# radhofan/Fairify

Measured on AMD Instinct MI355X. Metric: % partitions verified + partitions/sec on AC suite at 1/2/4/8 MI355X, higher is better.
Workload: dtype fp32

## Files before the change

fairify_amd/csrc/bindings.cpp:

```cpp
#include <hip/hip_runtime.h>
#include <pybind11/pybind11.h>
#include <pybind11/stl.h>

#include <cmath>
#include <cstring>
#include <cstdint>
#include <stdexcept>
#include <vector>

#include "runtime_host.h"

namespace py = pybind11;

extern "C" int fa_bounds_launch(const NetDesc& net, BoundArgs args, hipStream_t stream);
extern "C" int fa_crown_phase_launch(const NetDesc& net, CrownPhaseArgs a, hipStream_t stream);
extern "C" size_t fa_crown_phase_bytes(const NetDesc& net);
extern "C" int fa_point_try_launch(const NetDesc& net, BoundArgs a, hipStream_t stream);
extern "C" int fa_forward_launch(const NetDesc& net, FwdArgs a, hipStream_t stream);
extern "C" int fa_sim_launch(const NetDesc& net, SimArgs a, hipStream_t stream);
extern "C" int fa_sim_shaped(const NetDesc& net);
extern "C" int fa_ascent_launch(const NetDesc& net, AscentArgs a, hipStream_t stream);
extern "C" int fa_certify_launch(CertArgs a, hipStream_t stream);
extern "C" int fa_falsify_launch(const NetDesc& net, FalsifyArgs a, hipStream_t stream);
extern "C" int fa_prune_masks_launch(const NetDesc& net, int P, const int* counts, const float* ub, int ub_stride,
// ... 317 lines not shown
    a.npa = (int)pa.size();
    for (size_t i = 0; i < pa.size(); ++i) a.pa_idx[i] = pa[i];
    a.values = P<const int64_t>(values);
    a.Pp = Pp;
    a.pairs = P<const int64_t>(pairs);
    a.nfree = (int)free_dims.size();
    for (size_t i = 0; i < free_dims.size(); ++i) a.free_idx[i] = free_dims[i];
    a.found = P<uint8_t>(found);
    a.wit_x = P<float>(wit_x);
    a.wit_xp = P<float>(wit_xp);
    const int rc = fa_ascent_launch(net.d, a, (hipStream_t)stream);
    if (rc == -1) return false;
    ckl(rc, "ascent");
    return true;
  });

  m.def("falsify", [](const Net& net, uintptr_t flat, uintptr_t lo, uintptr_t hi, uintptr_t pids, int Pn,
                      int n_samples, int n_local, uint32_t seed, int V, const std::vector<int>& pa, uintptr_t values,
                      int Pp, uintptr_t pairs, int walk_k, int walk_steps, int K, int iters,
                      const std::vector<int>& free_dims, uintptr_t found, uintptr_t wit_x, uintptr_t wit_xp,
                      uintptr_t how, uintptr_t stream, const std::vector<int>& ra, int tau, uint32_t dseed) {
    if (pa.size() > FA_MAX_PA || free_dims.size() > 64 || ra.size() > FA_MAX_RA)
      throw std::invalid_argument("too many PA/RA/free dims");
    FalsifyArgs a{};
    a.flat = P<const float>(flat);
    a.lo = P<const float>(lo);
    a.hi = P<const float>(hi);
    a.pids = P<const int64_t>(pids);
    a.P = Pn; a.n_samples = n_samples; a.n_local = n_local; a.seed = seed;
    a.V = V;
    a.npa = (int)pa.size();
    for (size_t i = 0; i < pa.size(); ++i) a.pa_idx[i] = pa[i];
    a.values = P<const int64_t>(values);
    a.Pp = Pp;
    a.pairs = P<const int64_t>(pairs);
    a.walk_k = walk_k; a.walk_steps = walk_steps; a.K = K; a.iters = iters;
    a.nfree = (int)free_dims.size();
    for (size_t i = 0; i < free_dims.size(); ++i) a.free_idx[i] = free_dims[i];
    a.found = P<uint8_t>(found);
    a.wit_x = P<float>(wit_x);
    a.wit_xp = P<float>(wit_xp);
    a.how = P<int8_t>(how);
    a.nra = tau > 0 ? (int)ra.size() : 0;
    for (int i = 0; i < a.nra; ++i) a.ra_idx[i] = ra[i];
    a.tau = tau;
    a.dseed = dseed;
    const int rc = fa_falsify_launch(net.d, a, (hipStream_t)stream);
    if (rc == 0) return false;
    if (rc < 0) ckl(-rc, "falsify");
    return true;
  });

  m.def("prune_masks", [](const Net& net, int Pn, uintptr_t counts, uintptr_t ub, int ub_stride, uintptr_t sym_dead,
                          uintptr_t code, uintptr_t cnt, uintptr_t stream) {
    ckl(fa_prune_masks_launch(net.d, Pn, P<const int>(counts), P<const float>(ub), ub_stride,
                                P<const uint8_t>(sym_dead), P<uint8_t>(code), P<int>(cnt), (hipStream_t)stream),
          "prune_masks");
  });

  m.def("heuristic", [](const Net& net, int Pu, uintptr_t rows, uintptr_t lb, uintptr_t ub, int stride, uintptr_t code,
                        double q50, double qlo, double qhi, uintptr_t hnew, uintptr_t hmerged, uintptr_t hcnt,
                        uintptr_t stream) {
    ckl(fa_heuristic_launch(net.d, Pu, P<const int64_t>(rows), P<const float>(lb), P<const float>(ub), stride,
                              P<const uint8_t>(code), q50, qlo, qhi, P<uint8_t>(hnew), P<uint8_t>(hmerged),
                              P<int>(hcnt), (hipStream_t)stream),
          "heuristic");
  });

  m.def("agree", [](const Net& net, uintptr_t flat, int Pm, uintptr_t rows, uintptr_t lo, uintptr_t hi, uintptr_t pids,
                    uintptr_t dead, int S, uint32_t seed, uintptr_t agree, uintptr_t stream) {
    const int rc = fa_agree_launch(net.d, P<const float>(flat), Pm, P<const int64_t>(rows), P<const float>(lo),
                                   P<const float>(hi), P<const int64_t>(pids), P<const uint8_t>(dead), S, seed,
                                   P<int>(agree), (hipStream_t)stream);
    if (rc == 0) return false;
    if (rc < 0) ckl(-rc, "agree");
    return true;
  });

  m.def("certify", [](int Nn, int n0, int V, int Pp, int norient, std::vector<uintptr_t> fx, std::vector<uintptr_t> fxp,
                      uintptr_t xlo, uintptr_t xhi, uintptr_t xplo, uintptr_t xphi, uintptr_t pairs, uintptr_t values,
                      const std::vector<int>& pa, const std::vector<int>& ra, double tau, uintptr_t shared,
                      double unit, double gmarg, uintptr_t gmin, uintptr_t tstar, uintptr_t open, uintptr_t score,
                      uintptr_t split_dim, uintptr_t cand_x, uintptr_t cand_xp, uintptr_t cand_v, uintptr_t cand_o,
                      uintptr_t scores, uintptr_t leaf, uintptr_t stream) {
    if (pa.size() > FA_CMAX_PA || ra.size() > FA_MAX_RA) throw std::invalid_argument("too many PA/RA dims");
    if (fx.size() != 8 || fxp.size() != 8) throw std::invalid_argument("need 8 form pointers (6 forms + lb/ub)");
    CertArgs a{};
    a.Nn = Nn; a.n0 = n0; a.V = V; a.Pp = Pp; a.norient = norient;
    a.Lc = P<const float>(fx[0]); a.L0 = P<const float>(fx[1]); a.Le = P<const float>(fx[2]);
    a.Uc = P<const float>(fx[3]); a.U0 = P<const float>(fx[4]); a.Ue = P<const float>(fx[5]);
    a.olb = P<const float>(fx[6]); a.oub = P<const float>(fx[7]);
    a.Lcp = P<const float>(fxp[0]); a.L0p = P<const float>(fxp[1]); a.Lep = P<const float>(fxp[2]);
    a.Ucp = P<const float>(fxp[3]); a.U0p = P<const float>(fxp[4]); a.Uep = P<const float>(fxp[5]);
    a.olbp = P<const float>(fxp[6]); a.oubp = P<const float>(fxp[7]);
    a.xlo = P<const float>(xlo); a.xhi = P<const float>(xhi);
    a.xplo = P<const float>(xplo); a.xphi = P<const float>(xphi);
    a.pairs = P<const int64_t>(pairs);
    a.values = P<const int64_t>(values);
    a.npa = (int)pa.size();
    for (size_t i = 0; i < pa.size(); ++i) a.pa_idx[i] = pa[i];
    a.nra = (int)ra.size();
    for (size_t i = 0; i < ra.size(); ++i) a.ra_idx[i] = ra[i];
    a.tau = (float)tau;
    a.shared = P<const uint8_t>(shared);
    a.unit = (float)unit;
    a.gmarg = std::nextafter((float)gmarg, INFINITY);
    a.gmin = P<float>(gmin); a.tstar = P<float>(tstar);
    a.open = P<uint8_t>(open); a.score = P<float>(score); a.split_dim = P<int64_t>(split_dim);
    a.cand_x = P<float>(cand_x); a.cand_xp = P<float>(cand_xp);
    a.cand_v = P<int64_t>(cand_v); a.cand_o = P<int64_t>(cand_o);
    a.scores = P<float>(scores); a.leaf = P<uint8_t>(leaf);
    ckl(fa_certify_launch(a, (hipStream_t)stream), "certify");
  });

  m.def("decode", [](std::vector<int> radix, std::vector<long long> div, std::vector<int> chunk_off,
                     std::vector<float> base_lo, std::vector<float> base_hi, uintptr_t ids, int Pn,
                     uintptr_t chunk_lo, uintptr_t chunk_hi, uintptr_t lo, uintptr_t hi, uintptr_t stream) {
    const size_t n0 = radix.size();
    if (n0 == 0 || n0 > FA_DECODE_MAX_DIMS || div.size() != n0 || chunk_off.size() != n0 || base_lo.size() != n0 ||
        base_hi.size() != n0)
      throw std::invalid_argument("decode: descriptor sizes");
    DecodeDesc d{};
    d.n0 = (int)n0;
    for (size_t k = 0; k < n0; ++k) {
      if (radix[k] < 0 || (radix[k] > 0 && div[k] <= 0)) throw std::invalid_argument("decode: radix/div");
      d.radix[k] = radix[k];
      d.div[k] = div[k];
      d.chunk_off[k] = chunk_off[k];
      d.base_lo[k] = base_lo[k];
      d.base_hi[k] = base_hi[k];
    }
    ckl(fa_decode_launch(d, P<const int64_t>(ids), Pn, P<const float>(chunk_lo), P<const float>(chunk_hi),
                           P<float>(lo), P<float>(hi), (hipStream_t)stream),
          "decode");
  });
  m.def("pack_masks", [](uintptr_t src, int Pn, int N, int stride, int sel, uintptr_t out, int NB, uintptr_t hash,
                         uintptr_t stream) {
    ckl(fa_pack_masks_launch(P<const uint8_t>(src), Pn, N, stride, sel, P<uint8_t>(out), NB,
                               P<unsigned long long>(hash), (hipStream_t)stream),
          "pack_masks");
  });
  m.def("knn", [](uintptr_t X, int n, int d, int k, uintptr_t idx, uintptr_t dist, uintptr_t stream) {
    ckl(fa_knn_launch(P<const float>(X), n, d, k, P<int>(idx), P<float>(dist), (hipStream_t)stream), "knn");
  });
  m.def("actdiff", [](const Net& net, uintptr_t flat, uintptr_t x, uintptr_t xp, int npairs, uintptr_t sum_out,
                      uintptr_t stream) {
    ckl(fa_actdiff_launch(net.d, P<const float>(flat), P<const float>(x), P<const float>(xp), npairs,
                            P<float>(sum_out), (hipStream_t)stream),
          "actdiff");
  });
  m.def("trace_marker", [](int tag, uintptr_t sink, uintptr_t stream) {
    ckl(fa_trace_marker_launch(tag, P<int>(sink), (hipStream_t)stream), "trace_marker");
  });
  auto beta_args = [](const Net& net, uintptr_t flat, uintptr_t wt, int R, const std::vector<int>& pa, uintptr_t lo,
                      uintptr_t hi, uintptr_t va, uintptr_t vb, uintptr_t LBA, uintptr_t UBA, uintptr_t LBB,
                      uintptr_t UBB, uintptr_t phA, uintptr_t phB, uintptr_t par, uintptr_t t, uintptr_t scratch,
                      int iters, float lr_a, float lr_b, float lr_t, float decay, int lookahead, int beta_pos,
                      int stall, uintptr_t bound, uintptr_t split, uintptr_t xstar, uintptr_t binit,
                      unsigned long long ramask, uintptr_t plo, uintptr_t phi, uintptr_t xpstar, uintptr_t gtie,
                      float tau, uintptr_t osg) {
    if (pa.size() > FA_MAX_PA) throw std::invalid_argument("beta_level: too many PA dims");
    for (size_t q = 0; q < pa.size(); ++q)
      if (pa[q] < 0 || pa[q] >= net.d.dims[0] || (q && pa[q] <= pa[q - 1]))
        throw std::invalid_argument("beta_level: PA dims must be increasing input indices");
    BetaArgs a;
    std::memset(&a, 0, sizeof(a));
    a.flat = P<const float>(flat);
    a.wt = P<const float>(wt);
    a.R = R;
    a.npa = (int)pa.size();
    for (size_t q = 0; q < pa.size(); ++q) a.pa_idx[q] = pa[q];
    a.lo = P<const float>(lo);
    a.hi = P<const float>(hi);
    a.va = P<const float>(va);
    a.vb = P<const float>(vb);
    a.LBA = P<const float>(LBA);
    a.UBA = P<const float>(UBA);
    a.LBB = P<const float>(LBB);
    a.UBB = P<const float>(UBB);
    a.phA = P<const int8_t>(phA);
    a.phB = P<const int8_t>(phB);
    a.par = P<float>(par);
    a.t = P<float>(t);
    a.scratch = P<float>(scratch);
    a.iters = iters;
    a.lr_a = lr_a;
    a.lr_b = lr_b;
    a.lr_t = lr_t;
    a.decay = decay;
    a.lookahead = lookahead;
    a.beta_pos = beta_pos;
    a.stall = stall & 1;
    a.pgap = (stall >> 1) & 3;
    a.feas = (stall >> 3) & 1;
// ... 113 lines not shown
```

fairify_amd/csrc/certify.hip:

```cpp
#include "args.h"

struct Form {
  const float* c;
  float c0;
  float fmag;
};

__device__ __forceinline__ bool fa_is_pa(const CertArgs& a, int d) {
  for (int k = 0; k < a.npa; ++k)
    if (a.pa_idx[k] == d) return true;
  return false;
}

__device__ __forceinline__ Form fa_fold(const CertArgs& a, const float* C, float c0, int v) {
  Form f;
  f.c = C;
  float contrib = 0.f, cmag = 0.f;
  for (int k = 0; k < a.npa; ++k) {
    const float t = C[a.pa_idx[k]] * (float)a.values[v * a.npa + k];
    contrib += t;
    cmag += fabsf(t);
  }
  f.c0 = c0 + contrib;
  f.fmag = cmag;
// ... 81 lines not shown
  float ca[NM], cb[NM], xl[NM], xh[NM], pl[NM], ph[NM];
  bool sh[NM], un[NM];
  float magA = fabsf(A.c0) + A.fmag, magB = fabsf(B.c0) + B.fmag;
#pragma unroll
  for (int i = 0; i < NM; ++i) {
    const bool v = i < n0 && !fa_is_pa(a, i);
    ca[i] = v ? sA * A.c[i] : 0.f;
    cb[i] = v ? sB * B.c[i] : 0.f;
    xl[i] = v ? xlp[i] : 0.f;
    xh[i] = v ? xhp[i] : 0.f;
    pl[i] = v ? plp[i] : 0.f;
    ph[i] = v ? php[i] : 0.f;
    sh[i] = v && a.shared[i];
    un[i] = v && !a.shared[i];
    magA += fabsf(ca[i]) * fmaxf(fabsf(xl[i]), fabsf(xh[i]));
    magB += fabsf(cb[i]) * fmaxf(fabsf(pl[i]), fabsf(ph[i]));
  }
  const float A0 = sA * A.c0, B0 = sB * B.c0;
  const float marg0 = 8.f * a.unit * (magA + magB);
  auto g_at = [&](float t) __attribute__((always_inline)) {
    float val = 0.f;
#pragma unroll
    for (int i = 0; i < NM; ++i) {
      const float cs = t * ca[i] + (1.f - t) * cb[i];
      const float c1 = t * ca[i], c2 = (1.f - t) * cb[i];
      const float vs = fmaxf(cs * xl[i], cs * xh[i]);
      const float vu = fmaxf(c1 * xl[i], c1 * xh[i]) + fmaxf(c2 * pl[i], c2 * ph[i]);
      val += sh[i] ? vs : (un[i] ? vu : 0.f);
    }
    return val + t * A0 + (1.f - t) * B0 + a.gmarg * (t * magA + (1.f - t) * magB) + marg0;
  };
  float best = g_at(0.f), bt = 0.f;
  {
    const float g1 = g_at(1.f);
    if (g1 < best) { best = g1; bt = 1.f; }
  }
  if constexpr (NM <= 16) {
#pragma unroll
    for (int i = 0; i < NM; ++i) {
      if (!sh[i]) continue;
      const float den = ca[i] - cb[i];
      if (den == 0.f) continue;
      const float t = -cb[i] / den;
      if (!(t > 0.f && t < 1.f)) continue;
      const float g = g_at(t);
      if (g < best) { best = g; bt = t; }
    }
  } else {
#pragma unroll 1
    for (int i = 0; i < n0; ++i) {
      float ai = 0.f, bi = 0.f;
      bool s_i = false;
#pragma unroll
      for (int k = 0; k < NM; ++k)
        if (k == i) { ai = ca[k]; bi = cb[k]; s_i = sh[k]; }
      if (!s_i) continue;
      const float den = ai - bi;
      if (den == 0.f) continue;
      const float t = -bi / den;
      if (!(t > 0.f && t < 1.f)) continue;
      const float g = g_at(t);
      if (g < best) { best = g; bt = t; }
    }
  }
  gmin = best;
  tstar = bt;
}

template <int NM>
__global__ void __launch_bounds__(FA_CERT_THREADS) fa_pair_eval_kernel(CertArgs a) {
  const int Q = a.Pp * a.norient;
  const int64_t idx = (int64_t)blockIdx.x * FA_CERT_THREADS + threadIdx.x;
  if (idx >= (int64_t)a.Nn * Q) return;
  float g = -INFINITY, t = 0.f;
  const int n = (int)(idx / Q);
  const int8_t st = a.status ? a.status[a.part[n]] : (int8_t)3;
  if (st == 3 || st == 4) fa_pair_eval_one<NM>(a, n, (int)(idx % Q), g, t);
  a.gmin[idx] = g;
  a.tstar[idx] = t;
}

template <int NM>
__device__ __forceinline__ void fa_pick_node(const CertArgs& a, int n, float bg, int bq, float t);

template <int NM>
__global__ void __launch_bounds__(FA_CERT_THREADS) fa_pair_pick_kernel(CertArgs a) {
  const int n = blockIdx.x * FA_CERT_THREADS + threadIdx.x;
  if (n >= a.Nn) return;
  const int Q = a.Pp * a.norient;
  float bg = -INFINITY;
  int bq = 0;
  for (int qq = 0; qq < Q; ++qq) {
    float g = a.gmin[(size_t)n * Q + qq];
    if (g != g) g = INFINITY;
    if (g > bg) { bg = g; bq = qq; }
  }
  fa_pick_node<NM>(a, n, bg, bq, a.tstar[(size_t)n * Q + bq]);
}

#ifndef FA_CERT_WPE16
#define FA_CERT_WPE16 1
#endif
template <int NM>
__global__ void __launch_bounds__(FA_CERT_THREADS) __attribute__((amdgpu_waves_per_eu(NM == 16 ? FA_CERT_WPE16 : 1)))
fa_pair_fused_kernel(CertArgs a, int QG) {
  const int Q = a.Pp * a.norient;
  const int gidx = blockIdx.x * FA_CERT_THREADS + threadIdx.x;
  const int n = gidx / QG, qq = gidx - n * QG;
  bool live = n < a.Nn && qq < Q;
  if (live && a.status) {
    const int8_t st = a.status[a.part[n]];
    live = st == 3 || st == 4;
  }
  float g = -INFINITY, t = 0.f;
  if (live) fa_pair_eval_one<NM>(a, n, qq, g, t);
  if (g != g) g = INFINITY;
  int bq = live ? qq : 0x7fffffff;
  for (int o = 1; o < QG; o <<= 1) {
    const float g2 = __shfl_xor(g, o);
    const float t2 = __shfl_xor(t, o);
    const int q2 = __shfl_xor(bq, o);
    if (g2 > g || (g2 == g && q2 < bq)) { g = g2; t = t2; bq = q2; }
  }
  if (n < a.Nn && qq == 0) fa_pick_node<NM>(a, n, g, bq == 0x7fffffff ? 0 : bq, t);
}

template <int NM>
__device__ __forceinline__ void fa_pick_node(const CertArgs& a, int n, float bg, int bq, float t) {
  if (a.skip_closed && !(bg > 0.f)) {
    a.open[n] = 0;
    a.score[n] = bg;
    if (a.leaf) a.leaf[n] = 0;
    return;
  }
  const int o = bq / a.Pp, q = bq % a.Pp;
  Form A, B;
  float sA, sB;
  fa_pair_forms(a, n, q, o, A, sA, B, sB);
  const int n0 = a.n0;
  const float* xlp = a.xlo + (size_t)n * n0;
  const float* xhp = a.xhi + (size_t)n * n0;
  const float* plp = a.xplo + (size_t)n * n0;
  const float* php = a.xphi + (size_t)n * n0;
  float* cxo = a.cand_x + (size_t)n * n0;
  float* cpo = a.cand_xp + (size_t)n * n0;
  float* sco = a.scores ? a.scores + (size_t)n * 2 * n0 : nullptr;
  float ai[NM], bi[NM], xl[NM], xh[NM], pl[NM], ph[NM];
  unsigned pam = 0u, shm = 0u;
  for (int k = 0; k < a.npa; ++k) pam |= 1u << a.pa_idx[k];
#pragma unroll
  for (int i = 0; i < NM; ++i) {
    const bool v = i < n0;
    if (v && a.shared[i]) shm |= 1u << i;
    const bool p = (pam >> i) & 1u;
    ai[i] = (v && !p) ? sA * A.c[i] : 0.f;
    bi[i] = (v && !p) ? sB * B.c[i] : 0.f;
    xl[i] = v ? xlp[i] : 0.f;
    xh[i] = v ? xhp[i] : 0.f;
    pl[i] = v ? plp[i] : 0.f;
    ph[i] = v ? php[i] : 0.f;
  }
  float bs = -1.f;
  int bd = 0;
  bool leaf = true;
#pragma unroll
  for (int i = 0; i < NM; ++i) {
    if (i >= n0) continue;
    const float wx = xh[i] - xl[i];
    const float cs = t * ai[i] + (1.f - t) * bi[i];
    float sx, cx;
    if (((shm >> i) & 1u)) {
      sx = fabsf(cs) * wx;
      cx = cs > 0.f ? xh[i] : xl[i];
    } else {
      sx = fabsf(t * ai[i]) * wx;
      cx = (t * ai[i] > 0.f) ? xh[i] : xl[i];
    }
    sx += 1e-9f * wx;
    if (((pam >> i) & 1u) || wx <= 0.f) sx = -1.f;
    if (!((pam >> i) & 1u) && wx > 0.f) leaf = false;
    if (sx > bs) { bs = sx; bd = i; }
    if (sco) sco[i] = sx;
    cxo[i] = cx;
    cpo[i] = ((shm >> i) & 1u) ? cx : (((1.f - t) * bi[i] > 0.f) ? ph[i] : pl[i]);
  }
#pragma unroll
  for (int i = 0; i < NM; ++i) {
    if (i >= n0) continue;
    float sxp = -1.f;
    if (!((shm >> i) & 1u) && !((pam >> i) & 1u)) {
      const float wxp = ph[i] - pl[i];
      if (wxp > 0.f) {
        sxp = fabsf((1.f - t) * bi[i]) * wxp + 1e-9f * wxp;
        leaf = false;
      }
    }
    if (sco) sco[n0 + i] = sxp;
    if (sxp > bs) { bs = sxp; bd = n0 + i; }
  }
  if (a.smear && sco && a.nra == 0 && n0 <= NM) {
    float acc[NM];
#pragma unroll
    for (int i = 0; i < NM; ++i) acc[i] = 0.f;
    for (int v = 0; v < a.V; ++v) {
      const float* lb = a.lay_lb + ((size_t)n * a.V + v) * a.lay_N;
      const float* ub = a.lay_ub + ((size_t)n * a.V + v) * a.lay_N;
      for (int j0 = 0; j0 < a.n1; j0 += 32) {
        unsigned msk = 0u;
#pragma unroll
        for (int k = 0; k < 32; ++k) {
          const int j = j0 + k;
          const bool jv = j < a.n1;
          const float l = jv ? lb[j] : 0.f, u = jv ? ub[j] : 0.f;
          if (l < 0.f && u > 0.f) msk |= 1u << k;
        }
        while (msk) {
          int jj[2];
#pragma unroll
          for (int k = 0; k < 2; ++k) {
            jj[k] = msk ? j0 + __builtin_ctz(msk) : -1;
            msk &= msk - 1u;
          }
          float4 w[2][NM / 4];
#pragma unroll
          for (int k = 0; k < 2; ++k) {
            const float4* wr = reinterpret_cast<const float4*>(a.W0T + (size_t)(jj[k] < 0 ? 0 : jj[k]) * NM);
#pragma unroll
            for (int i4 = 0; i4 < NM / 4; ++i4) w[k][i4] = wr[i4];
          }
#pragma unroll
          for (int k = 0; k < 2; ++k) {
            if (jj[k] < 0) break;
#pragma unroll
            for (int i4 = 0; i4 < NM / 4; ++i4) {
              acc[4 * i4] += w[k][i4].x;
              acc[4 * i4 + 1] += w[k][i4].y;
              acc[4 * i4 + 2] += w[k][i4].z;
              acc[4 * i4 + 3] += w[k][i4].w;
            }
          }
        }
      }
    }
    bs = -1.f;
    bd = 0;
#pragma unroll
    for (int i = 0; i < NM; ++i) {
      if (i >= n0) continue;
      const float wx = xh[i] - xl[i];
      float sx = acc[i] * wx + 1e-9f * wx;
      if (((pam >> i) & 1u) || wx <= 0.f) sx = -1.f;
      sco[i] = sx;
      if (sx > bs) { bs = sx; bd = i; }
    }
  }
  const int vi = (int)a.pairs[2 * q], vj = (int)a.pairs[2 * q + 1];
  for (int k = 0; k < a.npa; ++k) {
    cxo[a.pa_idx[k]] = (float)a.values[vi * a.npa + k];
    cpo[a.pa_idx[k]] = (float)a.values[vj * a.npa + k];
  }
  for (int k = 0; k < a.nra; ++k) {
    const int r = a.ra_idx[k];
    const float v = fminf(fmaxf(cpo[r], cxo[r] - a.tau), cxo[r] + a.tau);
    cpo[r] = fminf(fmaxf(v, plp[r]), php[r]);
  }
  a.open[n] = bg > 0.f ? 1 : 0;
  a.score[n] = bg;
  a.split_dim[n] = bd;
  a.cand_v[n] = q;
  a.cand_o[n] = o;
  if (a.leaf) a.leaf[n] = leaf ? 1 : 0;
}

#ifndef FA_CERT_FUSE_Q
#define FA_CERT_FUSE_Q 4
#endif

extern "C" int fa_certify_launch(CertArgs a, hipStream_t stream) {
  if (a.Nn <= 0) return 0;
  if (a.npa > FA_CMAX_PA || a.nra > FA_MAX_RA) return -3;
  const int64_t tot = (int64_t)a.Nn * a.Pp * a.norient;
  if (a.Pp * a.norient <= FA_CERT_FUSE_Q && a.n0 <= 32) {
    int QG = 1;
    while (QG < a.Pp * a.norient) QG <<= 1;
    const dim3 gn((unsigned)(((int64_t)a.Nn * QG + FA_CERT_THREADS - 1) / FA_CERT_THREADS));
    if (a.n0 <= 16) hipLaunchKernelGGL(fa_pair_fused_kernel<16>, gn, dim3(FA_CERT_THREADS), 0, stream, a, QG);
    else hipLaunchKernelGGL(fa_pair_fused_kernel<32>, gn, dim3(FA_CERT_THREADS), 0, stream, a, QG);
    return (int)hipGetLastError();
  }
  const dim3 ge((unsigned)((tot + FA_CERT_THREADS - 1) / FA_CERT_THREADS));
  if (a.n0 <= 16) hipLaunchKernelGGL(fa_pair_eval_kernel<16>, ge, dim3(FA_CERT_THREADS), 0, stream, a);
  else if (a.n0 <= 32) hipLaunchKernelGGL(fa_pair_eval_kernel<32>, ge, dim3(FA_CERT_THREADS), 0, stream, a);
  else return -4;
  const dim3 gp((a.Nn + FA_CERT_THREADS - 1) / FA_CERT_THREADS);
  if (a.n0 <= 16) hipLaunchKernelGGL(fa_pair_pick_kernel<16>, gp, dim3(FA_CERT_THREADS), 0, stream, a);
  else hipLaunchKernelGGL(fa_pair_pick_kernel<32>, gp, dim3(FA_CERT_THREADS), 0, stream, a);
  return (int)hipGetLastError();
}
```

fairify_amd/ops/hip.py:

```python
from __future__ import annotations

import os
import threading
from typing import Optional, Sequence

import torch

from . import ext
from . import reference as ref


def _stream(dev) -> int:
    return torch.cuda.current_stream(dev).cuda_stream


_LAZY_LOCK = threading.Lock()


def _net(be):
    n = getattr(be, "_hipnet", None)
    if n is None:
        with _LAZY_LOCK:
            n = getattr(be, "_hipnet", None)
            if n is None:
# ... 212 lines not shown
    if res.lay_lb_full is None:
        raise ValueError("refine needs symbolic bounds with keep_layers=True (HIP layout)")
    lo = _c(lo, torch.float32, (R, n0), "lo")
    hi = _c(hi, torch.float32, (R, n0), "hi")
    d = None
    if dead is not None:
        d = _c(dead, torch.uint8, (R, be.n_hidden), "dead")
    ph = _c(phase, torch.int8, (R, be.n_hidden), "phase") if phase is not None else None
    infeas = torch.zeros(R, dtype=torch.uint8, device=lo.device) if phase is not None else None
    if R:
        ext().refine(_net(be), be.flat.data_ptr(), lo.data_ptr(), hi.data_ptr(), _ptr(d), R,
                     res.lay_lb_full.data_ptr(), res.lay_ub_full.data_ptr(), _stream(lo.device), _ptr(ph),
                     _ptr(infeas))
    if infeas is not None:
        res.infeasible = infeas.bool() if res.infeasible is None else (res.infeasible | infeas.bool())
    Nh = be.n_hidden
    if Nh:
        res.dead = res.lay_ub_full[:, :Nh] <= 0
        res.dead_u8 = res.dead.to(torch.uint8)
        res.active = res.lay_lb_full[:, :Nh] >= 0
    return res


def backward_bounds(be, lo: torch.Tensor, hi: torch.Tensor, dead: Optional[torch.Tensor] = None,
                    keep_layers: bool = True) -> Optional[ref.BoundResult]:
    R, n0 = lo.shape
    dev = lo.device
    lo = _c(lo, torch.float32, (R, n0), "lo")
    hi = _c(hi, torch.float32, (R, n0), "hi")
    f32 = dict(dtype=torch.float32, device=dev)
    res = ref.BoundResult(out_lb=torch.empty(R, **f32), out_ub=torch.empty(R, **f32),
                          Lc=torch.empty(R, n0, **f32), L0=torch.empty(R, **f32), Le=torch.empty(R, **f32),
                          Uc=torch.empty(R, n0, **f32), U0=torch.empty(R, **f32), Ue=torch.empty(R, **f32))
    N = be.mlp.n_neurons
    lay_lb = torch.empty(R, N, **f32) if keep_layers else None
    lay_ub = torch.empty(R, N, **f32) if keep_layers else None
    d = None
    if dead is not None:
        d = _c(dead, torch.uint8, (R, be.n_hidden), "dead")
    if R:
        rc = ext().backward_bounds(_net(be), be.flat.data_ptr(), lo.data_ptr(), hi.data_ptr(), _ptr(d), R,
                                   res.out_lb.data_ptr(), res.out_ub.data_ptr(), res.Lc.data_ptr(), res.L0.data_ptr(),
                                   res.Le.data_ptr(), res.Uc.data_ptr(), res.U0.data_ptr(), res.Ue.data_ptr(),
                                   _ptr(lay_lb), _ptr(lay_ub), _stream(dev))
        if rc == -1:
            return None
    if keep_layers:
        widths = be.mlp.widths
        offs = [0]
        for w in widths:
            offs.append(offs[-1] + w)
        res.layer_lb = [lay_lb[:, offs[i]:offs[i + 1]] for i in range(len(widths))]
        res.layer_ub = [lay_ub[:, offs[i]:offs[i + 1]] for i in range(len(widths))]
        res.lay_lb_full, res.lay_ub_full = lay_lb, lay_ub
        Nh = be.n_hidden
        res.dead = lay_ub[:, :Nh] <= 0
        if d is not None:
            res.dead = res.dead | d.bool()
        res.active = (lay_lb[:, :Nh] >= 0) & ~res.dead
    return res


def crown_phase(be, lo: torch.Tensor, hi: torch.Tensor, res: ref.BoundResult, phase: Optional[torch.Tensor] = None):
    R, n0 = lo.shape
    dev = lo.device
    lo = _c(lo, torch.float32, (R, n0), "lo")
    hi = _c(hi, torch.float32, (R, n0), "hi")
    if res.lay_lb_full is None:
        raise ValueError("crown_phase needs bounds(..., keep_layers=True) from the HIP path")
    ph = _c(phase, torch.int8, (R, be.n_hidden), "phase") if phase is not None else None
    split = torch.full((R, 2), -1, dtype=torch.int32, device=dev)
    score = torch.zeros(R, 2, dtype=torch.float32, device=dev)
    low = torch.zeros(R, 2, dtype=torch.float32, device=dev)
    infeas = res.infeasible.to(torch.uint8).contiguous() if res.infeasible is not None else None
    if R:
        ext().crown_phase(_net(be), be.flat.data_ptr(), lo.data_ptr(), hi.data_ptr(), R, _ptr(ph),
                          res.lay_lb_full.data_ptr(), res.lay_ub_full.data_ptr(), _ptr(infeas),
                          res.out_lb.data_ptr(), res.out_ub.data_ptr(), res.Lc.data_ptr(), res.L0.data_ptr(),
                          res.Le.data_ptr(), res.Uc.data_ptr(), res.U0.data_ptr(), res.Ue.data_ptr(),
                          split.data_ptr(), score.data_ptr(), low.data_ptr(), _stream(dev))
    return ref.PhaseCrown(low=low, split=split.long(), score=score), None


def pair_certify(be, res_x, res_xp, xlo, xhi, xplo, xphi, pairs, values, pa, shared, relaxed) -> ref.PairDecision:
    Nn, n0 = xlo.shape
    dev = xlo.device
    V = values.shape[0]
    Pp = pairs.shape[0]
    norient = 2 if relaxed else 1
    f32 = dict(dtype=torch.float32, device=dev)
    xlo = _c(xlo, torch.float32, (Nn, n0), "xlo")
    xhi = _c(xhi, torch.float32, (Nn, n0), "xhi")
    xplo = _c(xplo, torch.float32, (Nn, n0), "xplo")
    xphi = _c(xphi, torch.float32, (Nn, n0), "xphi")
    for r in (res_x, res_xp):
        if r.Lc is None or tuple(r.Lc.shape) != (Nn * V, n0):
            raise ValueError("pair_certify needs symbolic forms for Nn*V rows")
    pairs_c = _c(pairs, torch.int64, (Pp, 2), "pairs")
    values_c = _c(values, torch.int64, None, "values")
    sh = _c(shared, torch.uint8, (n0,), "shared")
    Q = Pp * norient
    gmin = torch.empty(Nn, Q, **f32)
    tstar = torch.empty(Nn, Q, **f32)
    open_ = torch.empty(Nn, dtype=torch.uint8, device=dev)
    score = torch.empty(Nn, **f32)
    split = torch.empty(Nn, dtype=torch.int64, device=dev)
    cx = torch.empty(Nn, n0, **f32)
    cxp = torch.empty(Nn, n0, **f32)
    cv = torch.empty(Nn, dtype=torch.int64, device=dev)
    co = torch.empty(Nn, dtype=torch.int64, device=dev)
    fx = [res_x.Lc, res_x.L0, res_x.Le, res_x.Uc, res_x.U0, res_x.Ue, res_x.out_lb, res_x.out_ub]
    fxp = [res_xp.Lc, res_xp.L0, res_xp.Le, res_xp.Uc, res_xp.U0, res_xp.Ue, res_xp.out_lb, res_xp.out_ub]
    fx = [_c(t, torch.float32) for t in fx]
    fxp = [_c(t, torch.float32) for t in fxp]
    scores = torch.empty(Nn, 2 * n0, **f32)
    leaf = torch.empty(Nn, dtype=torch.uint8, device=dev)
    if Nn:
        ext().certify(Nn, n0, V, Pp, norient, [t.data_ptr() for t in fx], [t.data_ptr() for t in fxp],
                      xlo.data_ptr(), xhi.data_ptr(), xplo.data_ptr(), xphi.data_ptr(), pairs_c.data_ptr(),
                      values_c.data_ptr(), [int(i) for i in pa.tolist()], [], 0.0, sh.data_ptr(), be.unit,
                      ref.gamma(2 * n0 + 4, be.unit), gmin.data_ptr(), tstar.data_ptr(), open_.data_ptr(),
                      score.data_ptr(), split.data_ptr(), cx.data_ptr(), cxp.data_ptr(), cv.data_ptr(),
                      co.data_ptr(), scores.data_ptr(), leaf.data_ptr(), _stream(dev))
    return ref.PairDecision(open_=open_.bool(), score=score, split_dim=split, cand_x=cx, cand_xp=cxp,
                            cand_v=cv, cand_orient=co)


def _parse_sim_blocks(v: Optional[str]) -> int:
    if v is None or v.strip() == "":
        return 0
    try:
        n = int(v)
    except ValueError:
        raise ValueError(f"FAIRIFY_SIM_BLOCKS={v!r}: expected a non-negative integer") from None
    if n < 0:
        raise ValueError(f"FAIRIFY_SIM_BLOCKS={v!r}: expected a non-negative integer")
    return n


_SIM_BLOCKS = _parse_sim_blocks(os.environ.get("FAIRIFY_SIM_BLOCKS"))
_SIM_BLOCKS_ENV: Optional[str] = None


def _sim_split(P: int, n_samples: int) -> int:
    target = _SIM_BLOCKS if _SIM_BLOCKS_ENV is None else _parse_sim_blocks(os.environ.get("FAIRIFY_SIM_BLOCKS"))
    if not P or target <= P:
        return 1
    tiles = (n_samples + 63) // 64
    return max(1, min(tiles, -(-target // P)))


_SIM_REGCOUNT = os.environ.get("FAIRIFY_SIM_REGCOUNT", "1").strip() != "0"
_SIM_REGCOUNT_ENV: Optional[str] = None


def _sim_regcount() -> bool:
    if _SIM_REGCOUNT_ENV is None:
        return _SIM_REGCOUNT
    return os.environ.get("FAIRIFY_SIM_REGCOUNT", "1").strip() != "0"


def simulate(be, q, lo, hi, pids, n_samples, seed, values, pairs, bisect_pairs, bisect_steps, return_z0=False):
    from ..engine.sim import SimResult, boundary_walk

    P, n0 = lo.shape
    dev = lo.device
    lo_c = _c(lo, torch.float32, (P, n0), "lo")
    hi_c = _c(hi, torch.float32, (P, n0), "hi")
    pids_c = _c(pids, torch.int64, (P,), "pids")
    V = values.shape[0]
    Pp = pairs.shape[0]
    values_c = _c(values, torch.int64, None, "values")
    pairs_c = _c(pairs, torch.int64, (Pp, 2), "pairs")
    split = _sim_split(P, n_samples)
    counts = (torch.zeros if split > 1 else torch.empty)(P, be.mlp.n_neurons, dtype=torch.int32, device=dev)
    keys = torch.full((P,), 0x7FFFFFFF, dtype=torch.int32, device=dev) if split > 1 else None
    found = torch.zeros(P, dtype=torch.uint8, device=dev)
    wx = torch.zeros(P, n0, dtype=torch.float32, device=dev)
    wxp = torch.zeros(P, n0, dtype=torch.float32, device=dev)
    walk = bool(bisect_pairs and bisect_steps)
    z0 = torch.empty(P, n_samples, dtype=torch.float32, device=dev) if (walk or return_z0) else None
    if P and n_samples:
        ext().sim(_net(be), be.flat.data_ptr(), lo_c.data_ptr(), hi_c.data_ptr(), pids_c.data_ptr(), P, n_samples,
                  int(seed) & 0xFFFFFFFF, V, list(q.pa_idx), values_c.data_ptr(), Pp, pairs_c.data_ptr(),
                  list(q.ra_idx) if q.relaxed else [], int(q.tau), counts.data_ptr(), found.data_ptr(),
                  wx.data_ptr(), wxp.data_ptr(), _ptr(z0), _ptr(keys), split, int(_sim_regcount()), _stream(dev))
    res = SimResult(counts=counts, found=found.bool(), wit_x=wx, wit_xp=wxp)
    if return_z0:
        res.z0 = z0
    if walk:
        boundary_walk(be, q, lo_c, hi_c, pids_c, n_samples, seed, values_c, pairs_c, res, z0, bisect_pairs,
                      bisect_steps)
    return res


def ascent(be, q, lo, hi, x0, f0, q0, iters, values, pairs, free_dims):
    P, K, n0 = x0.shape
    dev = x0.device
    lo_c = _c(lo, torch.float32, (P, n0), "lo")
    hi_c = _c(hi, torch.float32, (P, n0), "hi")
    x0_c = _c(x0, torch.float32, (P, K, n0), "x0")
    f0_c = _c(f0, torch.float32, (P, K), "f0")
    q0_c = _c(q0, torch.int32, (P, K), "q0")
    V = values.shape[0]
    Pp = pairs.shape[0]
    values_c = _c(values, torch.int64, None, "values")
# ... 334 lines not shown
```

Measured before the change: 272,000.

## Add wave-cooperative group pick with LDS-staged weights and optional smear scoring

```diff
diff --git a/fairify_amd/csrc/bindings.cpp b/fairify_amd/csrc/bindings.cpp
--- a/fairify_amd/csrc/bindings.cpp
+++ b/fairify_amd/csrc/bindings.cpp
@@ -423,7 +423,14 @@
                       const std::vector<int>& pa, const std::vector<int>& ra, double tau, uintptr_t shared,
                       double unit, double gmarg, uintptr_t gmin, uintptr_t tstar, uintptr_t open, uintptr_t score,
                       uintptr_t split_dim, uintptr_t cand_x, uintptr_t cand_xp, uintptr_t cand_v, uintptr_t cand_o,
-                      uintptr_t scores, uintptr_t leaf, uintptr_t stream) {
+                      uintptr_t scores, uintptr_t leaf, uintptr_t stream, py::args opt) {
+    if (opt.size() > 4) throw std::invalid_argument("certify: at most 4 optional arguments");
+    const int skip_closed = opt.size() > 0 ? opt[0].cast<int>() : 0;
+    const uintptr_t status = opt.size() > 1 ? opt[1].cast<uintptr_t>() : 0;
+    const uintptr_t part = opt.size() > 2 ? opt[2].cast<uintptr_t>() : 0;
+    const std::vector<uintptr_t> smear = opt.size() > 3 ? opt[3].cast<std::vector<uintptr_t>>() : std::vector<uintptr_t>();
+    if ((status != 0) != (part != 0)) throw std::invalid_argument("certify: status and part go together");
+    if (!smear.empty() && smear.size() != 5) throw std::invalid_argument("certify: smear needs 5 entries");
     if (pa.size() > FA_CMAX_PA || ra.size() > FA_MAX_RA) throw std::invalid_argument("too many PA/RA dims");
     if (fx.size() != 8 || fxp.size() != 8) throw std::invalid_argument("need 8 form pointers (6 forms + lb/ub)");
     CertArgs a{};
@@ -451,6 +458,13 @@
     a.cand_x = P<float>(cand_x); a.cand_xp = P<float>(cand_xp);
     a.cand_v = P<int64_t>(cand_v); a.cand_o = P<int64_t>(cand_o);
     a.scores = P<float>(scores); a.leaf = P<uint8_t>(leaf);
+    a.skip_closed = skip_closed;
+    a.status = P<const int8_t>(status); a.part = P<const int>(part);
+    if (!smear.empty()) {
+      a.smear = 1;
+      a.lay_lb = P<const float>(smear[0]); a.lay_ub = P<const float>(smear[1]); a.lay_N = (int)smear[2];
+      a.W0T = P<const float>(smear[3]); a.n1 = (int)smear[4];
+    }
     ckl(fa_certify_launch(a, (hipStream_t)stream), "certify");
   });
 
diff --git a/fairify_amd/csrc/certify.hip b/fairify_amd/csrc/certify.hip
--- a/fairify_amd/csrc/certify.hip
+++ b/fairify_amd/csrc/certify.hip
@@ -187,28 +187,40 @@
 
 template <int NM>
 __device__ __forceinline__ void fa_pick_node(const CertArgs& a, int n, float bg, int bq, float t);
-
-template <int NM>
+template <int NM>
+__device__ __forceinline__ void fa_pick_wave(const CertArgs& a, float* w0s, bool need, int n, float bg, int bq,
+                                             float t);
+#ifndef FA_CERT_W0_LDS
+#define FA_CERT_W0_LDS 4096
+#endif
+
+template <int NM, bool GP>
 __global__ void __launch_bounds__(FA_CERT_THREADS) fa_pair_pick_kernel(CertArgs a) {
+  __shared__ __attribute__((aligned(16))) float w0s[GP ? FA_CERT_W0_LDS : 4];
   const int n = blockIdx.x * FA_CERT_THREADS + threadIdx.x;
-  if (n >= a.Nn) return;
+  const bool in = n < a.Nn;
+  if (!GP && !in) return;
   const int Q = a.Pp * a.norient;
   float bg = -INFINITY;
   int bq = 0;
-  for (int qq = 0; qq < Q; ++qq) {
-    float g = a.gmin[(size_t)n * Q + qq];
-    if (g != g) g = INFINITY;
-    if (g > bg) { bg = g; bq = qq; }
-  }
-  fa_pick_node<NM>(a, n, bg, bq, a.tstar[(size_t)n * Q + bq]);
+  if (in)
+    for (int qq = 0; qq < Q; ++qq) {
+      float g = a.gmin[(size_t)n * Q + qq];
+      if (g != g) g = INFINITY;
+      if (g > bg) { bg = g; bq = qq; }
+    }
+  const float t = in ? a.tstar[(size_t)n * Q + bq] : 0.f;
+  if constexpr (GP) fa_pick_wave<NM>(a, w0s, in, n, bg, bq, t);
+  else fa_pick_node<NM>(a, n, bg, bq, t);
 }
 
 #ifndef FA_CERT_WPE16
 #define FA_CERT_WPE16 1
 #endif
-template <int NM>
+template <int NM, bool GP>
 __global__ void __launch_bounds__(FA_CERT_THREADS) __attribute__((amdgpu_waves_per_eu(NM == 16 ? FA_CERT_WPE16 : 1)))
 fa_pair_fused_kernel(CertArgs a, int QG) {
+  __shared__ __attribute__((aligned(16))) float w0s[GP ? FA_CERT_W0_LDS : 4];
   const int Q = a.Pp * a.norient;
   const int gidx = blockIdx.x * FA_CERT_THREADS + threadIdx.x;
   const int n = gidx / QG, qq = gidx - n * QG;
@@ -227,7 +239,8 @@
     const int q2 = __shfl_xor(bq, o);
     if (g2 > g || (g2 == g && q2 < bq)) { g = g2; t = t2; bq = q2; }
   }
-  if (n < a.Nn && qq == 0) fa_pick_node<NM>(a, n, g, bq == 0x7fffffff ? 0 : bq, t);
+  if constexpr (GP) fa_pick_wave<NM>(a, w0s, n < a.Nn && qq == 0, n, g, bq == 0x7fffffff ? 0 : bq, t);
+  else if (n < a.Nn && qq == 0) fa_pick_node<NM>(a, n, g, bq == 0x7fffffff ? 0 : bq, t);
 }
 
 template <int NM>
@@ -377,6 +390,238 @@
   if (a.leaf) a.leaf[n] = leaf ? 1 : 0;
 }
 
+struct FaPickIn {
+  bool act;
+  int n, o, q, vi, vj;
+  float bg, t;
+  float ai, bi, xl, xh, pl, ph;
+};
+
+template <int NM>
+__device__ __forceinline__ FaPickIn fa_pick_load(const CertArgs& a, bool act, int n, float bg, int bq, float t,
+                                                 int vi, int vj) {
+  FaPickIn r;
+  const int i = threadIdx.x & (NM - 1);
+  const int n0 = a.n0;
+  const bool v = act && i < n0;
+  r.act = act; r.n = n; r.bg = bg; r.t = t;
+  r.o = bq / a.Pp; r.q = bq % a.Pp;
+  r.vi = vi; r.vj = vj;
+  const size_t ri = (size_t)n * a.V + r.vi, rj = (size_t)n * a.V + r.vj;
+  const float* Ac = (r.o == 0 ? a.Lc : a.Uc) + ri * n0;
+  const float* Bc = (r.o == 0 ? a.Ucp : a.Lcp) + rj * n0;
+  const float sA = r.o == 0 ? -1.f : 1.f, sB = r.o == 0 ? 1.f : -1.f;
+  const size_t e = (size_t)n * n0 + i;
+  bool p = false;
+  for (int k = 0; k < a.npa; ++k) p |= a.pa_idx[k] == i;
+  r.ai = (v && !p) ? sA * Ac[i] : 0.f;
+  r.bi = (v && !p) ? sB * Bc[i] : 0.f;
+  r.xl = v ? a.xlo[e] : 0.f; r.xh = v ? a.xhi[e] : 0.f;
+  r.pl = v ? a.xplo[e] : 0.f; r.ph = v ? a.xphi[e] : 0.f;
+  return r;
+}
+
+template <int NM>
+__device__ __forceinline__ void fa_pick_group(const CertArgs& a, const float* w0s, int w0p, const FaPickIn& in) {
+#pragma clang fp contract(off)
+  constexpr unsigned long long GM = NM == 32 ? 0xffffffffull : 0xffffull;
+  const int lane = threadIdx.x & 63;
+  const int i = lane & (NM - 1), gsh = (lane / NM) * NM;
+  const int n0 = a.n0;
+  const bool act = in.act;
+  const int n = in.n, o = in.o, q = in.q, vi = in.vi, vj = in.vj;
+  const float bg = in.bg, t = in.t;
+  const bool v = act && i < n0;
+  const size_t e = (size_t)n * n0 + i;
+  bool p = false;
+  for (int k = 0; k < a.npa; ++k) p |= a.pa_idx[k] == i;
+  const bool sh = v && a.shared[i];
+  const float ai = in.ai, bi = in.bi, xl = in.xl, xh = in.xh, pl = in.pl, ph = in.ph;
+  const float wx = xh - xl;
+  const float ta = t * ai, ub = (1.f - t) * bi;
+  const float cs = ta + ub;
+  float sx, cx;
+  if (sh) {
+    sx = fabsf(cs) * wx;
+    cx = cs > 0.f ? xh : xl;
+  } else {
+    sx = fabsf(ta) * wx;
+    cx = (ta > 0.f) ? xh : xl;
+  }
+  sx += 1e-9f * wx;
+  if (p || wx <= 0.f) sx = -1.f;
+  bool inner = !p && wx > 0.f;
+  float cp = sh ? cx : ((ub > 0.f) ? ph : pl);
+  float sxp = -1.f;
+  if (!sh && !p) {
+    const float wxp = ph - pl;
+    if (wxp > 0.f) {
+      sxp = fabsf(ub) * wxp + 1e-9f * wxp;
+      inner = true;
+    }
+  }
+  if (!v) { sx = -1.f; sxp = -1.f; inner = false; }
+  const bool smear = a.smear && a.scores && a.nra == 0 && n0 <= NM;
+  if (smear) {
+    constexpr int CH = 512 / (2 * NM);
+    float acc = 0.f;
+    const int tot = a.V * ((a.n1 + NM - 1) / NM);
+    int cv = 0, cj = 0;
+    for (int c0 = 0; c0 < tot; c0 += CH) {
+      float l[CH], u[CH];
+      int jb[CH];
+      {
+        int v2 = cv, j2 = cj;
+#pragma unroll
+        for (int c = 0; c < CH; ++c) {
+          const bool cvld = c0 + c < tot;
+          const int j = j2 + i;
+          const bool jv = act && cvld && j < a.n1;
+          const size_t off = ((size_t)n * a.V + v2) * a.lay_N + j;
+          l[c] = jv ? a.lay_lb[off] : 0.f;
+          u[c] = jv ? a.lay_ub[off] : 0.f;
+          jb[c] = j2;
+          j2 += NM;
+          if (j2 >= a.n1) { j2 = 0; ++v2; }
+        }
+        cv = v2;
+        cj = j2;
+      }
+#pragma unroll
+      for (int c = 0; c < CH; ++c) {
+        if (c0 + c >= tot) break;
+        const unsigned long long bm = __ballot(l[c] < 0.f && u[c] > 0.f);
+        if (!bm) continue;
+        const unsigned msk = (unsigned)((bm >> gsh) & GM);
+        const float4* wr = reinterpret_cast<const float4*>(w0s + i * w0p + jb[c]);
+#pragma unroll
+        for (int k4 = 0; k4 < NM / 4; ++k4) {
+          const float4 w = wr[k4];
+          acc += ((msk >> (4 * k4)) & 1u) ? w.x : 0.f;
+          acc += ((msk >> (4 * k4 + 1)) & 1u) ? w.y : 0.f;
+          acc += ((msk >> (4 * k4 + 2)) & 1u) ? w.z : 0.f;
+          acc += ((msk >> (4 * k4 + 3)) & 1u) ? w.w : 0.f;
+        }
+      }
+    }
+    sx = acc * wx + 1e-9f * wx;
+    if (p || wx <= 0.f) sx = -1.f;
+    if (!v) sx = -1.f;
+  }
+  float bs = -1.f;
+  int bd = 0x7fffffff;
+  if (sx > -1.f) { bs = sx; bd = i; }
+  if (!smear && sxp > bs) { bs = sxp; bd = n0 + i; }
+#pragma unroll
+  for (int w = NM / 2; w > 0; w >>= 1) {
+    const float s2 = __shfl_xor(bs, w);
+    const int d2 = __shfl_xor(bd, w);
+    if (s2 > bs || (s2 == bs && d2 < bd)) { bs = s2; bd = d2; }
+  }
+  if (bd == 0x7fffffff) bd = 0;
+  const bool leaf = ((__ballot(inner) >> gsh) & GM) == 0ull;
+  if (p)
+    for (int k = 0; k < a.npa; ++k)
+      if (a.pa_idx[k] == i) {
+        cx = (float)a.values[vi * a.npa + k];
+        cp = (float)a.values[vj * a.npa + k];
+      }
+  for (int k = 0; k < a.nra; ++k)
+    if (a.ra_idx[k] == i) {
+      const float c2 = fminf(fmaxf(cp, cx - a.tau), cx + a.tau);
+      cp = fminf(fmaxf(c2, pl), ph);
+    }
+  if (v) {
+    if (a.scores) {
+      float* sco = a.scores + (size_t)n * 2 * n0;
+      sco[i] = sx;
+      sco[n0 + i] = sxp;
+    }
+    a.cand_x[e] = cx;
+    a.cand_xp[e] = cp;
+  }
+  if (act && i == 0) {
+    a.open[n] = bg > 0.f ? 1 : 0;
+    a.score[n] = bg;
+    a.split_dim[n] = bd;
+    a.cand_v[n] = q;
+    a.cand_o[n] = o;
+    if (a.leaf) a.leaf[n] = leaf ? 1 : 0;
+  }
+}
+
+template <int NM>
+__device__ __forceinline__ void fa_pick_wave(const CertArgs& a, float* w0s, bool need, int n, float bg, int bq,
+                                             float t) {
+  if (need && a.skip_closed && !(bg > 0.f)) {
+    a.open[n] = 0;
+    a.score[n] = bg;
+    if (a.leaf) a.leaf[n] = 0;
+    need = false;
+  }
+  unsigned long long m = __ballot(need);
+  if (!m) return;
+  int vi = 0, vj = 0;
+  if (need) {
+    const int q = bq % a.Pp;
+    vi = (int)a.pairs[2 * q];
+    vj = (int)a.pairs[2 * q + 1];
+  }
+  const int lane = threadIdx.x & 63;
+  const int grp = lane / NM;
+  int w0p = 0;
+  if (a.smear && a.scores && a.nra == 0 && a.n0 <= NM) {
+    const int pitch = (a.n1 + NM - 1) / NM * NM + 4;
+    {
+      const int tot4 = a.n1 * NM / 4;
+      const float4* src4 = reinterpret_cast<const float4*>(a.W0T);
+      for (int b = 0; b < tot4; b += 8 * FA_CERT_THREADS) {
+        float4 w[8];
+#pragma unroll
+        for (int u = 0; u < 8; ++u) {
+          const int k4 = b + u * FA_CERT_THREADS + lane;
+          w[u] = k4 < tot4 ? src4[k4] : make_float4(0.f, 0.f, 0.f, 0.f);
+        }
+#pragma unroll
+        for (int u = 0; u < 8; ++u) {
+          const int k4 = b + u * FA_CERT_THREADS + lane;
+          if (k4 < tot4) {
+            float* d = w0s + ((4 * k4) & (NM - 1)) * pitch + (4 * k4) / NM;
+            d[0] = w[u].x; d[pitch] = w[u].y; d[2 * pitch] = w[u].z; d[3 * pitch] = w[u].w;
+          }
+        }
+      }
+      __syncthreads();
+      w0p = pitch;
+    }
+  }
+  auto take = [&]() __attribute__((always_inline)) {
+    int src = -1;
+#pragma unroll
+    for (int k = 0; k < 64 / NM; ++k) {
+      if (m && k == grp) src = __builtin_ctzll(m);
+      m &= m - 1ull;
+    }
+    const bool act = src >= 0;
+    const int s = act ? src : 0;
+    const int n2 = __shfl(n, s), q2 = __shfl(bq, s);
+    const float g2 = __shfl(bg, s), t2 = __shfl(t, s);
+    const int vi2 = __shfl(vi, s), vj2 = __shfl(vj, s);
+    return fa_pick_load<NM>(a, act, act ? n2 : 0, g2, act ? q2 : 0, t2, act ? vi2 : 0, act ? vj2 : 0);
+  };
+  FaPickIn cur0 = take(), cur1 = take();
+  for (;;) {
+    const bool more = m != 0ull;
+    FaPickIn nxt0 = cur0, nxt1 = cur1;
+    if (more) { nxt0 = take(); nxt1 = take(); }
+    fa_pick_group<NM>(a, w0s, w0p, cur0);
+    if (__ballot(cur1.act)) fa_pick_group<NM>(a, w0s, w0p, cur1);
+    if (!more) break;
+    cur0 = nxt0;
+    cur1 = nxt1;
+  }
+}
+
 #ifndef FA_CERT_FUSE_Q
 #define FA_CERT_FUSE_Q 4
 #endif
@@ -385,20 +630,42 @@
   if (a.Nn <= 0) return 0;
   if (a.npa > FA_CMAX_PA || a.nra > FA_MAX_RA) return -3;
   const int64_t tot = (int64_t)a.Nn * a.Pp * a.norient;
-  if (a.Pp * a.norient <= FA_CERT_FUSE_Q && a.n0 <= 32) {
+  const bool fused = a.Pp * a.norient <= FA_CERT_FUSE_Q && a.n0 <= 32;
+  const bool smear = a.smear && a.scores && a.nra == 0;
+  bool gp = a.n0 <= 16 && (fused || smear);
+  if (const char* e = getenv("FAIRIFY_CERT_GROUP_PICK")) {
+    if (*e == '0') gp = false;
+    if (*e == '1') gp = a.n0 <= 32;
+  }
+  if (gp && smear) {
+    const int nm = a.n0 <= 16 ? 16 : 32;
+    if (nm * ((a.n1 + nm - 1) / nm * nm + 4) > FA_CERT_W0_LDS) gp = false;
+  }
+  if (fused) {
     int QG = 1;
     while (QG < a.Pp * a.norient) QG <<= 1;
     const dim3 gn((unsigned)(((int64_t)a.Nn * QG + FA_CERT_THREADS - 1) / FA_CERT_THREADS));
-    if (a.n0 <= 16) hipLaunchKernelGGL(fa_pair_fused_kernel<16>, gn, dim3(FA_CERT_THREADS), 0, stream, a, QG);
-    else hipLaunchKernelGGL(fa_pair_fused_kernel<32>, gn, dim3(FA_CERT_THREADS), 0, stream, a, QG);
+    const dim3 bt(FA_CERT_THREADS);
+    if (a.n0 <= 16) {
+      if (gp) hipLaunchKernelGGL((fa_pair_fused_kernel<16, true>), gn, bt, 0, stream, a, QG);
+      else hipLaunchKernelGGL((fa_pair_fused_kernel<16, false>), gn, bt, 0, stream, a, QG);
+    } else {
+      if (gp) hipLaunchKernelGGL((fa_pair_fused_kernel<32, true>), gn, bt, 0, stream, a, QG);
+      else hipLaunchKernelGGL((fa_pair_fused_kernel<32, false>), gn, bt, 0, stream, a, QG);
+    }
     return (int)hipGetLastError();
   }
   const dim3 ge((unsigned)((tot + FA_CERT_THREADS - 1) / FA_CERT_THREADS));
   if (a.n0 <= 16) hipLaunchKernelGGL(fa_pair_eval_kernel<16>, ge, dim3(FA_CERT_THREADS), 0, stream, a);
   else if (a.n0 <= 32) hipLaunchKernelGGL(fa_pair_eval_kernel<32>, ge, dim3(FA_CERT_THREADS), 0, stream, a);
   else return -4;
-  const dim3 gp((a.Nn + FA_CERT_THREADS - 1) / FA_CERT_THREADS);
-  if (a.n0 <= 16) hipLaunchKernelGGL(fa_pair_pick_kernel<16>, gp, dim3(FA_CERT_THREADS), 0, stream, a);
-  else hipLaunchKernelGGL(fa_pair_pick_kernel<32>, gp, dim3(FA_CERT_THREADS), 0, stream, a);
+  const dim3 gk((a.Nn + FA_CERT_THREADS - 1) / FA_CERT_THREADS), bt(FA_CERT_THREADS);
+  if (a.n0 <= 16) {
+    if (gp) hipLaunchKernelGGL((fa_pair_pick_kernel<16, true>), gk, bt, 0, stream, a);
+    else hipLaunchKernelGGL((fa_pair_pick_kernel<16, false>), gk, bt, 0, stream, a);
+  } else {
+    if (gp) hipLaunchKernelGGL((fa_pair_pick_kernel<32, true>), gk, bt, 0, stream, a);
+    else hipLaunchKernelGGL((fa_pair_pick_kernel<32, false>), gk, bt, 0, stream, a);
+  }
   return (int)hipGetLastError();
 }
diff --git a/fairify_amd/ops/hip.py b/fairify_amd/ops/hip.py
--- a/fairify_amd/ops/hip.py
+++ b/fairify_amd/ops/hip.py
@@ -318,7 +318,16 @@
     return ref.PhaseCrown(low=low, split=split.long(), score=score), None
 
 
-def pair_certify(be, res_x, res_xp, xlo, xhi, xplo, xphi, pairs, values, pa, shared, relaxed) -> ref.PairDecision:
+def smear_w0t(be, n0: int) -> torch.Tensor:
+    nm = 16 if n0 <= 16 else 32
+    w0 = be.ws[0].detach().to(torch.float32)
+    wt = torch.zeros(w0.shape[1], nm, dtype=torch.float32, device=w0.device)
+    wt[:, :n0] = w0.abs().t()
+    return wt.contiguous()
+
+
+def pair_certify(be, res_x, res_xp, xlo, xhi, xplo, xphi, pairs, values, pa, shared, relaxed, *, ra=(), tau=0.0,
+                 skip_closed=False, status=None, part=None, smear=False, fill=None, raw=False):
     Nn, n0 = xlo.shape
     dev = xlo.device
     V = values.shape[0]
@@ -336,28 +345,57 @@
     values_c = _c(values, torch.int64, None, "values")
     sh = _c(shared, torch.uint8, (n0,), "shared")
     Q = Pp * norient
-    gmin = torch.empty(Nn, Q, **f32)
-    tstar = torch.empty(Nn, Q, **f32)
-    open_ = torch.empty(Nn, dtype=torch.uint8, device=dev)
-    score = torch.empty(Nn, **f32)
-    split = torch.empty(Nn, dtype=torch.int64, device=dev)
-    cx = torch.empty(Nn, n0, **f32)
-    cxp = torch.empty(Nn, n0, **f32)
-    cv = torch.empty(Nn, dtype=torch.int64, device=dev)
-    co = torch.empty(Nn, dtype=torch.int64, device=dev)
+
+    def buf(shape, dtype):
+        t = torch.empty(shape, dtype=dtype, device=dev)
+        if fill is not None:
+            t.view(torch.uint8).fill_(int(fill))
+        return t
+
+    gmin = buf((Nn, Q), torch.float32)
+    tstar = buf((Nn, Q), torch.float32)
+    open_ = buf((Nn,), torch.uint8)
+    score = buf((Nn,), torch.float32)
+    split = buf((Nn,), torch.int64)
+    cx = buf((Nn, n0), torch.float32)
+    cxp = buf((Nn, n0), torch.float32)
+    cv = buf((Nn,), torch.int64)
+    co = buf((Nn,), torch.int64)
     fx = [res_x.Lc, res_x.L0, res_x.Le, res_x.Uc, res_x.U0, res_x.Ue, res_x.out_lb, res_x.out_ub]
     fxp = [res_xp.Lc, res_xp.L0, res_xp.Le, res_xp.Uc, res_xp.U0, res_xp.Ue, res_xp.out_lb, res_xp.out_ub]
     fx = [_c(t, torch.float32) for t in fx]
     fxp = [_c(t, torch.float32) for t in fxp]
-    scores = torch.empty(Nn, 2 * n0, **f32)
-    leaf = torch.empty(Nn, dtype=torch.uint8, device=dev)
+    scores = buf((Nn, 2 * n0), torch.float32)
+    leaf = buf((Nn,), torch.uint8)
+    if (status is None) != (part is None):
+        raise ValueError("pair_certify: status and part go together")
+    st = _c(status, torch.int8, None, "status") if status is not None else None
+    pt = _c(part, torch.int32, (Nn,), "part") if part is not None else None
+    sm = []
+    if smear:
+        if n0 > 32:
+            raise ValueError("pair_certify: smear scores need n0 <= 32")
+        if res_x.lay_lb_full is None or res_x.lay_lb_full.shape[0] != Nn * V:
+            raise ValueError("pair_certify: smear needs bounds(..., keep_layers=True) of the x rows")
+        lay_lb = _c(res_x.lay_lb_full, torch.float32)
+        lay_ub = _c(res_x.lay_ub_full, torch.float32)
+        w0t = smear_w0t(be, n0)
+        sm = [lay_lb.data_ptr(), lay_ub.data_ptr(), int(lay_lb.shape[1]), w0t.data_ptr(), int(w0t.shape[0])]
+    args = (Nn, n0, V, Pp, norient, [t.data_ptr() for t in fx], [t.data_ptr() for t in fxp],
+            xlo.data_ptr(), xhi.data_ptr(), xplo.data_ptr(), xphi.data_ptr(), pairs_c.data_ptr(),
+            values_c.data_ptr(), [int(i) for i in pa.tolist()], [int(i) for i in ra], float(tau),
+            sh.data_ptr(), be.unit,
+            ref.gamma(2 * n0 + 4, be.unit), gmin.data_ptr(), tstar.data_ptr(), open_.data_ptr(),
+            score.data_ptr(), split.data_ptr(), cx.data_ptr(), cxp.data_ptr(), cv.data_ptr(),
+            co.data_ptr(), scores.data_ptr(), leaf.data_ptr(), _stream(dev),
+            1 if skip_closed else 0, _ptr(st), _ptr(pt), sm)
     if Nn:
-        ext().certify(Nn, n0, V, Pp, norient, [t.data_ptr() for t in fx], [t.data_ptr() for t in fxp],
-                      xlo.data_ptr(), xhi.data_ptr(), xplo.data_ptr(), xphi.data_ptr(), pairs_c.data_ptr(),
-                      values_c.data_ptr(), [int(i) for i in pa.tolist()], [], 0.0, sh.data_ptr(), be.unit,
-                      ref.gamma(2 * n0 + 4, be.unit), gmin.data_ptr(), tstar.data_ptr(), open_.data_ptr(),
-                      score.data_ptr(), split.data_ptr(), cx.data_ptr(), cxp.data_ptr(), cv.data_ptr(),
-                      co.data_ptr(), scores.data_ptr(), leaf.data_ptr(), _stream(dev))
+        ext().certify(*args)
+    if raw:
+        keep = (args, fx, fxp, xlo, xhi, xplo, xphi, pairs_c, values_c, sh, gmin, tstar, st, pt,
+                sm and (lay_lb, lay_ub, w0t))
+        return dict(open=open_, score=score, split_dim=split, cand_x=cx, cand_xp=cxp, cand_v=cv, cand_o=co,
+                    scores=scores, leaf=leaf, relaunch=lambda _k=keep: ext().certify(*_k[0]))
     return ref.PairDecision(open_=open_.bool(), score=score, split_dim=split, cand_x=cx, cand_xp=cxp,
                             cand_v=cv, cand_orient=co)
 
```

Result: no change. 274,200, median of 2 (+0.8%).
